# inhavl-shlee/AFI-GAN

Hardware: AMD Instinct MI355X
Metric: stage1_G+D_step_images_per_s (higher is better)
Workload: dtype f32 via f16x3: two scaled fp16 pieces per operand, three f16 MFMAs per product, fp32 accumulate (tensors fp32)

## Files before the change

afigan_amd/_lib.py:

```python
import ctypes as C
import os

import torch

_HERE = os.path.dirname(os.path.abspath(__file__))
LIB_PATH = os.environ.get("AFI_LIB_PATH") or os.path.join(_HERE, "csrc", "libafigan_hip.so")

AFI_MAX_RDB = 8
ABI_VERSION = 8


class AfiError(RuntimeError):
    pass


class View(C.Structure):
    _fields_ = [("p", C.c_void_p), ("sN", C.c_longlong), ("sH", C.c_longlong), ("sW", C.c_longlong)]


class GenParams(C.Structure):
    _fields_ = [("C", C.c_int), ("G", C.c_int), ("n_rdb", C.c_int), ("residual_scale", C.c_float),
                ("w0", C.c_void_p), ("b0", C.c_void_p),
                ("rdb_w", (C.c_void_p * 5) * AFI_MAX_RDB),
                ("w7", C.c_void_p), ("b7", C.c_void_p),
# ... 59 lines not shown
    "afi_conv1x1_wgrad": (_i, [_vp, View, View, _i, _i, _i, _i, _i, _vp, _f, _vp]),
    "afi_conv3x3_wino_ws_floats": (_ll, [_i] * 5),
    "afi_conv3x3_wino_fwd": (_i, [_vp, View, _i, _i, _i, _i, _vp, _vp, _i, View, _vp, _ll, _vp]),
    "afi_conv3x3_wino_infer": (_i, [_vp, View, _i, _i, _i, _i, _vp, _vp, _i, View, _i, _vp, _ll, _vp]),
    "afi_conv3x3_wino_dgrad": (_i, [_vp, View, _i, _i, _i, _i, _vp, _i, View, View, _vp, _ll, _vp]),
    "afi_conv3x3_wino_wgrad": (_i, [_vp, View, View, _i, _i, _i, _i, _i, _vp, _f, _vp, _ll, _vp]),
    "afi_conv3x3s2_fwd": (_i, [_vp, View, _i, _i, _i, _i, _vp, _vp, _i, View, _i, View, _f, View, _f, _vp]),
    "afi_conv3x3s2_dgrad": (_i, [_vp, View, _i, _i, _i, _i, _vp, _i, View, _f, _f, _vp]),
    "afi_conv3x3s2_wgrad": (_i, [_vp, View, View, _i, _i, _i, _i, _i, _vp, _f, _vp]),
    "afi_relu_bwd": (_i, [_vp, _vp, _vp, _ll, _f, _vp]),
    "afi_dwconv3x3_fwd": (_i, [View, _i, _i, _i, _i, _vp, _vp, _vp]),
    "afi_maxpool3s2_same_fwd": (_i, [View, _i, _i, _i, _i, _vp, _vp]),
    "afi_fuse_swish_fwd": (_i, [_vp, _vp, _vp, _vp, _vp, _ll, _vp]),
    "afi_fuse_swish_bwd_scratch_floats": (_ll, []),
    "afi_fuse_swish_bwd": (_i, [_vp, _vp, _vp, _vp, _vp, _vp, _vp, _vp, _vp, _ll, _vp, _vp]),
    "afi_dwconv3x3_wgrad_scratch_floats": (_ll, [_i]),
    "afi_dwconv3x3_wgrad": (_i, [_vp, _vp, _i, _i, _i, _i, _vp, _vp, _vp]),
    "afi_maxpool3s2_same_fwd_idx": (_i, [View, _i, _i, _i, _i, _vp, _vp, _vp]),
    "afi_maxpool3s2_same_bwd": (_i, [_vp, _vp, _i, _i, _i, _i, _vp, _vp]),
    "afi_bn_stats_ex": (_i, [_vp, _ll, _i, _f, _f, _vp, _vp, _vp, _vp, _vp, _vp, _vp, _vp]),
    "afi_bn_apply_fwd": (_i, [_vp, _vp, _vp, _vp, _vp, _vp, _ll, _i, _f, _vp]),
    "afi_resize_bilinear_u8_ws_bytes": (_ll, [_i, _i, _i, _i, _i]),
    "afi_resize_bilinear_u8": (_i, [_vp, _i, _i, _i, _vp, _i, _i, _i, _i, _vp, _ll, _vp]),
    "afi_dual_scale_u8_ws_bytes": (_ll, [_i, _i, _i, _i, _i, _i, _i]),
    "afi_dual_scale_u8": (_i, [_vp, _i, _i, _i, _vp, _i, _i, _i, _vp, _i, _i, _i, _i, _vp, _ll, _vp]),
    "afi_normalize_pad_u8": (_i, [_vp, _i, _i, _i, _vp, _vp, _vp, _i, _i, _vp]),
    "afi_convT6s2_pack_weight": (_i, [_vp, _vp, _i, _i, _vp]),
    "afi_convT6s2_unpack_wgrad": (_i, [_vp, _vp, _i, _i, _vp]),
    "afi_convT6s2_fwd": (_i, [_vp, View, _i, _i, _i, _i, _vp, _vp, _i, View, _i, _vp]),
    "afi_convT6s2_dgrad": (_i, [_vp, View, _i, _i, _i, _i, _vp, _i, View, View, _vp]),
    "afi_convT6s2_wgrad": (_i, [_vp, View, View, _i, _i, _i, _i, _i, _vp, _f, _vp]),
    "afi_bilinear2x_add_fwd": (_i, [View, _i, _i, _i, _i, _f, _vp, _vp]),
    "afi_bilinear2x_add_bwd": (_i, [_vp, _i, _i, _i, _i, _f, _vp, _vp]),
    "afi_reduce_scratch_floats": (_ll, [_i]),
    "afi_bn_stats": (_i, [_vp, _ll, _i, _vp, _vp, _vp, _vp, _vp, _vp, _vp]),
    "afi_bn_apply_lrelu_fwd": (_i, [_vp, _vp, _vp, _vp, _vp, _vp, _ll, _i, _vp]),
    "afi_bn_bwd": (_i, [_vp, _vp, _vp, _vp, _vp, _vp, _vp, _vp, _ll, _i, _vp, _vp]),
    "afi_bn_bwd_sums": (_i, [_vp, _vp, _vp, _vp, _vp, _vp, _vp, _ll, _i, _vp, _vp]),
    "afi_bn_bwd_apply": (_i, [_vp, _vp, _vp, _vp, _vp, _vp, _vp, _ll, _ll, _i, _vp]),
    "afi_colsum_accum": (_i, [_vp, _ll, _i, _ll, _f, _vp, _vp, _vp]),
    "afi_bce_logits_fwd_bwd": (_i, [_vp, _ll, _f, _f, _vp, _f, _vp, _vp]),
    "afi_l1_fwd_bwd": (_i, [View, View, _i, _i, _i, _i, _i, _i, _f, _vp, _f, _vp, _vp]),
    "afi_sgd_momentum_step": (_i, [_vp, _i, _ll, _f, _f, _f, _vp]),
    "afi_scale_inplace": (_i, [_vp, _ll, _f, _vp]),
    "afi_nchw_to_nhwc": (_i, [_vp, _vp, _i, _i, _i, _vp]),
    "afi_nhwc_to_nchw": (_i, [_vp, _vp, _i, _i, _i, _vp]),
    "afi_profile_enable": (_i, [_i]),
    "afi_profile_num_kinds": (_i, []),
    "afi_profile_kind_name": (C.c_char_p, [_i]),
    "afi_profile_get": (_i, [_i, C.POINTER(C.c_double)]),
    "afi_profile_dump": (_i, [C.c_char_p]),
    "afi_debug_wk6_convT_images": (_i, [_vp, _i, _i, _i, _vp, _vp, _vp, _vp, C.POINTER(C.c_longlong), _vp]),
    "afi_debug_wgrad_sk_plan": (_i, [C.POINTER(C.c_longlong), C.POINTER(C.c_int), _i, _i, C.POINTER(C.c_int), C.POINTER(C.c_int), C.POINTER(C.c_int)]),
}

_lib = None


def load():
    global _lib
    if _lib is not None:
        return _lib
    if not os.path.exists(LIB_PATH):
        raise AfiError(f"{LIB_PATH} not found: build it with `python __graft_entry__.py` (hipcc --offload-arch=gfx950). "
                       "There is no CPU fallback for the AFI-GAN hot path.")
    lib = C.CDLL(LIB_PATH)
    for name, (res, args) in SIGNATURES.items():
        fn = getattr(lib, name)
        fn.restype = res
        fn.argtypes = args
    if lib.afi_abi_version() != ABI_VERSION:
        raise AfiError(f"ABI mismatch: library {lib.afi_abi_version()} != binding {ABI_VERSION}")
    if not os.environ.get("AFI_LIB_PATH"):
        want, have = tree_digest(), lib.afi_build_id().decode()
        if want is not None and have != want:
            raise AfiError(f"{LIB_PATH} was built from other sources than this tree (library {have[:16]}, tree {want[:16]}): "
                           "rebuild it with `python -c 'import __graft_entry__ as g; g.build()'`")
    _lib = lib
    return lib


def tree_digest():
    import glob
    import hashlib
    csrc = os.path.join(_HERE, "csrc")
    hdr = os.path.join(os.path.dirname(_HERE), "include", "afigan_hip.h")
    files = sorted(glob.glob(os.path.join(csrc, "*.hip")) + [f for f in glob.glob(os.path.join(csrc, "*.h")) if os.path.basename(f) != "afi_build_id.h"])
    if not files or not os.path.exists(hdr):
        return None
    h = hashlib.sha256()
    for f in files + [hdr]:
        h.update(os.path.basename(f).encode() + b"\0")
        h.update(open(f, "rb").read())
    return h.hexdigest()


def build_id():
    return load().afi_build_id().decode()


def check(status: int, what: str = ""):
    if status != 0:
        msg = load().afi_status_string(status).decode()
        raise AfiError(f"{what or 'afigan_hip call'} failed: status {status} ({msg})")


# ... 134 lines not shown
```

afigan_amd/csrc/afi_gemm_f16.h:

```cpp
#pragma once

#include "afi_f16_split.h"
__device__ __forceinline__ f16x8 afi_tr_frag_f16(const unsigned char* base, int off_lo, int off_hi) {
    return __builtin_bit_cast(f16x8, afi_tr_frag(base, off_lo, off_hi));
}

__device__ __forceinline__ float afi_wave_max(float m) {
#pragma unroll
    for (int o = 32; o > 0; o >>= 1) m = fmaxf(m, __shfl_xor(m, o));
    return m;
}
__device__ __forceinline__ void afi_block_amax_publish(float m, float* slot) {
    __shared__ float red[16];
    m = afi_wave_max(m);
    const int lane = threadIdx.x & 63, wave = threadIdx.x >> 6, nw = (blockDim.x + 63) >> 6;
    if (lane == 0) red[wave] = m;
    __syncthreads();
    if (threadIdx.x == 0) {
        for (int w = 1; w < nw; ++w) m = fmaxf(m, red[w]);
        const unsigned bits = __float_as_uint(m);
        const unsigned cur = __hip_atomic_load((const unsigned*)slot, __ATOMIC_RELAXED, __HIP_MEMORY_SCOPE_AGENT);
        if (bits > cur) (void)atomicMax((unsigned*)slot, bits);
    }
}
// ... 531 lines not shown
        for (int ni = 0; ni < NI; ++ni) {
            bh[ni] = afi_tr_frag_f16(cur, fb_off[ni][0], fb_off[ni][1]);
            bl[ni] = afi_tr_frag_f16(cur + PART, fb_off[ni][0], fb_off[ni][1]);
        }
#pragma unroll
        for (int ni = 0; ni < NI; ++ni)
#pragma unroll
            for (int mi = 0; mi < MI; ++mi) acc[mi][ni] = mm(al[mi], bh[ni], acc[mi][ni]);
#pragma unroll
        for (int ni = 0; ni < NI; ++ni)
#pragma unroll
            for (int mi = 0; mi < MI; ++mi) acc[mi][ni] = mm(ah[mi], bl[ni], acc[mi][ni]);
#pragma unroll
        for (int ni = 0; ni < NI; ++ni)
#pragma unroll
            for (int mi = 0; mi < MI; ++mi) acc[mi][ni] = mm(ah[mi], bh[ni], acc[mi][ni]);
        asm volatile("s_waitcnt lgkmcnt(0)" ::: "memory");
    }
    const bool use_atomic = gridDim.y > 1;
    float* out = p.dU + (long long)plane * p.M * p.N;
    const long long ldn = p.N;
    if (use_atomic) {
#pragma unroll
        for (int mi = 0; mi < MI; ++mi)
#pragma unroll
            for (int ni = 0; ni < NI; ++ni)
#pragma unroll
                for (int r = 0; r < 16; ++r) {
                    const int row = m0 + (wm * MI + mi) * 32 + (r & 3) + 8 * (r >> 2) + 4 * lh;
                    __builtin_amdgcn_global_atomic_fadd_f32((__attribute__((address_space(1))) float*)(out + (long long)row * ldn + n0 + (wn * NI + ni) * 32 + lr),
                                                            (acc[mi][ni][r] * inv_q) * inv_v);
                }
    } else {
#pragma unroll
        for (int mi = 0; mi < MI; ++mi) {
            float old[NI][16];
#pragma unroll
            for (int ni = 0; ni < NI; ++ni)
#pragma unroll
                for (int r = 0; r < 16; ++r) {
                    const int row = m0 + (wm * MI + mi) * 32 + (r & 3) + 8 * (r >> 2) + 4 * lh;
                    old[ni][r] = out[(long long)row * ldn + n0 + (wn * NI + ni) * 32 + lr];
                }
#pragma unroll
            for (int ni = 0; ni < NI; ++ni)
#pragma unroll
                for (int r = 0; r < 16; ++r) {
                    const int row = m0 + (wm * MI + mi) * 32 + (r & 3) + 8 * (r >> 2) + 4 * lh;
                    out[(long long)row * ldn + n0 + (wn * NI + ni) * 32 + lr] = old[ni][r] + (acc[mi][ni][r] * inv_q) * inv_v;
                }
        }
    }
}
```

afigan_amd/csrc/igemm.hip:

```cpp
#include "afi_common.h"

#define AFI_BK 32
#define AFI_LDK (AFI_BK + 4)


__device__ __attribute__((aligned(16))) float afi_zeros[4] = {0.f, 0.f, 0.f, 0.f};

#include "afi_epilogue.h"

template <bool POST>
__global__ __launch_bounds__(256) void afi_pix_splitk_epilogue_kernel(const AfiPixGemm p) {
    const int HW = p.H * p.W;
    const long long M = (long long)p.N * HW;
    const int ldp = (p.Ncols + 3) & ~3;
    const int C_F4 = ldp >> 2;
    const long long total = M * C_F4;
    for (long long it = (long long)blockIdx.x * 256 + threadIdx.x; it < total; it += (long long)gridDim.x * 256) {
        const long long m = it / C_F4;
        const int col = (int)(it - m * C_F4) * 4;
        f32x4 v = {0.f, 0.f, 0.f, 0.f};
        const float* src = p.partial + m * ldp + col;
        const long long slab = M * ldp;
        int ks = 0;
        for (; ks + 4 <= p.splitK; ks += 4) {
// ... 478 lines not shown
    const long long ldn = p.N;
    if (use_atomic) {
#pragma unroll
        for (int mi = 0; mi < MI; ++mi)
#pragma unroll
            for (int r = 0; r < 16; ++r) {
                const int row = m0 + MI * ((r & 3) + 8 * (r >> 2) + 4 * lh) + mi;
                atomicAdd(out + (long long)row * ldn + n0 + wn * 32 + lr, acc[mi][r]);
            }
    } else {
        float old[MI][16];
#pragma unroll
        for (int mi = 0; mi < MI; ++mi)
#pragma unroll
            for (int r = 0; r < 16; ++r) {
                const int row = m0 + MI * ((r & 3) + 8 * (r >> 2) + 4 * lh) + mi;
                old[mi][r] = out[(long long)row * ldn + n0 + wn * 32 + lr];
            }
#pragma unroll
        for (int mi = 0; mi < MI; ++mi)
#pragma unroll
            for (int r = 0; r < 16; ++r) {
                const int row = m0 + MI * ((r & 3) + 8 * (r >> 2) + 4 * lh) + mi;
                out[(long long)row * ldn + n0 + wn * 32 + lr] = old[mi][r] + acc[mi][r];
            }
    }
}

#include <vector>
#include <atomic>
#include <mutex>
namespace {
struct ProfRec { hipEvent_t a, b; int kind; double flops; long long m; int n, k, split, planes; };
struct ProfState {
    std::atomic<bool> on{false};
    std::mutex mu;
    std::vector<ProfRec> recs;
    std::vector<hipEvent_t> pool;
    size_t used = 0;
} g_prof;
const char* kKindNames[] = {
    "pix_gemm<128x128,KC,linear> (1x1 / ragged-map / non-aligned Winograd GEMMs)", "pix_gemm<128x64,KC>", "pix_gemm<128x32,KC>", "pix_gemm<64x64,KC>",
    "pix_gemm<128x128,RC,linear> (conv dgrad, mid-size / ragged maps)", "pix_gemm<128x64,RC>", "pix_gemm<128x32,RC>", "pix_gemm<64x64,RC>",
    "wgrad_gemm<128x128>", "wgrad_gemm<64x128>", "wgrad_gemm<32x128>",
    "pix_gemm<128x128,KC,halo> (conv fwd)", "pix_gemm<128x128,RC,halo> (conv dgrad)",
    "gemm_nt<128x128> (batched Winograd GEMM)", "gemm_tn<128x128> (Winograd weight-gradient GEMM)",
    "pix_gemm_wk (small-map pixel GEMM, K split inside the block; grouped launches included)",
    "wgrad_group (grouped weight gradients of a small-map backward pass)",
    "gemm_nt_bf16<128x128> (batched Winograd GEMM on the bf16 MFMA: bf16x6 / bf16x3 / bf16 operands, fp32 accumulate)",
    "gemm_tn_bf16<128x128> (Winograd weight-gradient GEMM on the bf16 MFMA: bf16x6 / bf16x3 / bf16 operands, fp32 accumulate)",
    "wgrad_group6 (grouped weight gradients of a small-map backward pass on the bf16 MFMA, bf16x6 operands, fp32 accumulate)",
    "pix_gemm_wk6 (small-map pixel GEMM on the bf16 MFMA, bf16x6 operands on pre-split weight images, fp32 accumulate; grouped launches included)",
    "gemm_nt_f16x3 (batched Winograd GEMM on the f16 MFMA, 256x256 tiles where the grid fills the chip and 128x128 below: two scaled fp16 pieces per operand, three products, fp32 accumulate)",
    "gemm_tn_f16x3<128x128> (Winograd weight-gradient GEMM on the f16 MFMA: two scaled fp16 pieces per operand, three products, fp32 accumulate)"};
constexpr int kNumKinds = 23;
hipEvent_t prof_event() {
    if (g_prof.used == g_prof.pool.size()) {
        hipEvent_t e;
        (void)hipEventCreate(&e);
        g_prof.pool.push_back(e);
    }
    return g_prof.pool[g_prof.used++];
}
struct ProfScope {
    hipStream_t st; int kind; double flops; hipEvent_t a{};
    long long m = 0; int n = 0, k = 0, split = 1, planes = 1;
    ProfScope(hipStream_t s, int kd, double f) : st(s), kind(kd), flops(f) {
        if (g_prof.on) { std::lock_guard<std::mutex> lk(g_prof.mu); a = prof_event(); (void)hipEventRecord(a, st); started = true; }
    }
    bool live = true, started = false;
    void cancel() { live = false; }
    ~ProfScope() {
        if (started && live) { std::lock_guard<std::mutex> lk(g_prof.mu); hipEvent_t b = prof_event(); (void)hipEventRecord(b, st); g_prof.recs.push_back({a, b, kind, flops, m, n, k, split, planes}); }
    }
};
}

extern "C" int afi_profile_enable(int on) {
    std::lock_guard<std::mutex> lk(g_prof.mu);
    if (on) { g_prof.recs.clear(); g_prof.used = 0; }
    g_prof.on = on != 0;
    return AFI_OK;
}
extern "C" int afi_profile_num_kinds(void) { return kNumKinds; }
extern "C" const char* afi_profile_kind_name(int kind) { return (kind >= 0 && kind < kNumKinds) ? kKindNames[kind] : ""; }
extern "C" int afi_profile_get(int kind, double* out) {
    out[0] = out[1] = out[2] = 0.0;
    for (const ProfRec& r : g_prof.recs) {
        if (r.kind != kind) continue;
        if (hipEventSynchronize(r.b) != hipSuccess) return AFI_ERR_LAUNCH;
        float ms = 0.f;
        if (hipEventElapsedTime(&ms, r.a, r.b) != hipSuccess) return AFI_ERR_LAUNCH;
        out[0] += 1.0; out[1] += ms; out[2] += r.flops;
    }
    return AFI_OK;
}

#include <stdio.h>
extern "C" int afi_profile_dump(const char* path) {
    FILE* f = fopen(path, "w");
    if (!f) return AFI_ERR_BAD_ARG;
    fprintf(f, "kind,rows,cols,k,split,planes,ms,tflops\n");
    for (const ProfRec& r : g_prof.recs) {
        float ms = 0.f;
        if (hipEventSynchronize(r.b) != hipSuccess || hipEventElapsedTime(&ms, r.a, r.b) != hipSuccess) { fclose(f); return AFI_ERR_LAUNCH; }
        fprintf(f, "\"%s\",%lld,%d,%d,%d,%d,%.4f,%.2f\n", kKindNames[r.kind], r.m, r.n, r.k, r.split, r.planes, ms, ms > 0.f ? r.flops / (ms * 1e-3) / 1e12 : 0.0);
    }
// ... 161 lines not shown
                             bool a_pre, long long nt256_min_tiles, bool local_sums) {
    if (planes <= 0 || planes > 36 || rows_per_plane <= 0 || N <= 0 || K <= 0 || !ab.amax) return AFI_ERR_BAD_ARG;
    if ((rows_per_plane % 128) || (N % 128) || (K % 32)) return AFI_ERR_UNSUPPORTED;
    AfiGemmNT g{A, (const float*)Bimg, C, rows_per_plane, planes, N, K};
    const long long M = rows_per_plane * planes;
    const int ntm = (int)(M / 128), ntn = N / 128, chunk = afi_cdiv(ntm, 8);
    const size_t stage = 16384u + 2u * 8192u, epi = sizeof(float) * 64u * (128u + 4u);
    const size_t lds = stage > epi ? stage : epi;
    ProfScope prof(st, 21, 2.0 * (double)M * N * K);
    prof.m = M; prof.n = N; prof.k = K; prof.split = 2; prof.planes = planes;
    const int tpp = afi_cdiv(rows_per_plane, 256);
    const long long tiles256 = (long long)planes * tpp * (N / 256);
    if (local_sums && a_pre && !(N % 256)) {
        if (!afi_opt_in_big_lds((const void*)afi_gemm_nt_f16x3_w16_kernel<true, true>)) return AFI_ERR_LAUNCH;
        const int ntm2 = planes * tpp, ntn2 = N / 256, chunk2 = afi_cdiv(ntm2, 8);
        prof.split = 7;
        hipLaunchKernelGGL((afi_gemm_nt_f16x3_w16_kernel<true, true>), dim3(chunk2 * ntn2 * 8), dim3(1024), 16 * 16 * 132 * 4, st, g, ab, ntn2, ntm2, chunk2, tpp);
        return hipGetLastError() == hipSuccess ? AFI_OK : AFI_ERR_LAUNCH;
    }
    if (nt256_min_tiles > 0 && !(g_nt_abl & 32) && !(N % 256) && tiles256 >= nt256_min_tiles) {
        if (!afi_opt_in_big_lds(a_pre ? (const void*)afi_gemm_nt_f16x3_w16_kernel<true> : (const void*)afi_gemm_nt_f16x3_w16_kernel<false>)) return AFI_ERR_LAUNCH;
        const int ntm2 = planes * tpp, ntn2 = N / 256, chunk2 = afi_cdiv(ntm2, 8);
        prof.split = a_pre ? 4 : 3;
        if (a_pre) hipLaunchKernelGGL(afi_gemm_nt_f16x3_w16_kernel<true>, dim3(chunk2 * ntn2 * 8), dim3(1024), 16 * 16 * 132 * 4, st, g, ab, ntn2, ntm2, chunk2, tpp);
        else hipLaunchKernelGGL(afi_gemm_nt_f16x3_w16_kernel<false>, dim3(chunk2 * ntn2 * 8), dim3(1024), 16 * 16 * 132 * 4, st, g, ab, ntn2, ntm2, chunk2, tpp);
        return hipGetLastError() == hipSuccess ? AFI_OK : AFI_ERR_LAUNCH;
    }
    if (a_pre) {
        prof.split = 5;
        hipLaunchKernelGGL((afi_gemm_nt_f16x3_kernel<4, 0, true>), dim3(chunk * ntn * 8), dim3(256), lds, st, g, ab, ntn, ntm, chunk);
        return hipGetLastError() == hipSuccess ? AFI_OK : AFI_ERR_LAUNCH;
    }
#ifdef AFI_ABLATIONS
    const int abl = g_nt_abl & 31;
    if (abl == 1) hipLaunchKernelGGL((afi_gemm_nt_f16x3_kernel<4, 1>), dim3(chunk * ntn * 8), dim3(256), lds, st, g, ab, ntn, ntm, chunk);
    else if (abl == 2) hipLaunchKernelGGL((afi_gemm_nt_f16x3_kernel<4, 2>), dim3(chunk * ntn * 8), dim3(256), lds, st, g, ab, ntn, ntm, chunk);
    else if (abl == 4) hipLaunchKernelGGL((afi_gemm_nt_f16x3_kernel<4, 4>), dim3(chunk * ntn * 8), dim3(256), lds, st, g, ab, ntn, ntm, chunk);
    else if (abl == 8) hipLaunchKernelGGL((afi_gemm_nt_f16x3_kernel<4, 8>), dim3(chunk * ntn * 8), dim3(256), lds, st, g, ab, ntn, ntm, chunk);
    else if (abl == 16) hipLaunchKernelGGL((afi_gemm_nt_f16x3_kernel<4, 16>), dim3(chunk * ntn * 8), dim3(256), lds, st, g, ab, ntn, ntm, chunk);
    else if (abl == 12) hipLaunchKernelGGL((afi_gemm_nt_f16x3_kernel<4, 12>), dim3(chunk * ntn * 8), dim3(256), lds, st, g, ab, ntn, ntm, chunk);
    else if (abl == 6) hipLaunchKernelGGL((afi_gemm_nt_f16x3_kernel<4, 6>), dim3(chunk * ntn * 8), dim3(256), lds, st, g, ab, ntn, ntm, chunk);
    else if (abl == 14) hipLaunchKernelGGL((afi_gemm_nt_f16x3_kernel<4, 14>), dim3(chunk * ntn * 8), dim3(256), lds, st, g, ab, ntn, ntm, chunk);
    else if (abl == 10) hipLaunchKernelGGL((afi_gemm_nt_f16x3_kernel<4, 10>), dim3(chunk * ntn * 8), dim3(256), lds, st, g, ab, ntn, ntm, chunk);
    else if (abl == 20) hipLaunchKernelGGL((afi_gemm_nt_f16x3_kernel<4, 20>), dim3(chunk * ntn * 8), dim3(256), lds, st, g, ab, ntn, ntm, chunk);
    else if (abl == 24) hipLaunchKernelGGL((afi_gemm_nt_f16x3_kernel<4, 24>), dim3(chunk * ntn * 8), dim3(256), lds, st, g, ab, ntn, ntm, chunk);
    else
#endif
    hipLaunchKernelGGL((afi_gemm_nt_f16x3_kernel<4>), dim3(chunk * ntn * 8), dim3(256), lds, st, g, ab, ntn, ntm, chunk);
    return hipGetLastError() == hipSuccess ? AFI_OK : AFI_ERR_LAUNCH;
}
#ifndef AFI_TN_MAX_ROUNDS
#define AFI_TN_MAX_ROUNDS 6
#endif
int afi_launch_gemm_tn_f16x3(const float* Q, const float* V, float* dU, int planes, long long rows_per_plane, int M, int N, const AfiF16Bound& qb, const AfiF16Bound& vb,
                             hipStream_t st, bool pre, bool deterministic) {
    if (planes <= 0 || planes > 36 || rows_per_plane <= 0 || M <= 0 || N <= 0 || !qb.amax || !vb.amax) return AFI_ERR_BAD_ARG;
    if ((rows_per_plane % 32) || (M % 128) || (N % 128)) return AFI_ERR_UNSUPPORTED;
    const int ntm = M / 128, ntn = N / 128;
    const long long tiles = (long long)ntm * ntn * planes;
    const int slots = AFI_TN_WAVES == 8 ? 768 : (AFI_TN_RING == 3 ? 768 : (AFI_TN_RING == 2 ? 1024 : 512));
    int splitK = 1;
    {
        const int maxsplit = (int)(rows_per_plane / (16 * 32)) > 0 ? (int)(rows_per_plane / (16 * 32)) : 1;
        double best = -1.0;
        for (int s2 = 1; s2 <= maxsplit && s2 <= 128; ++s2) {
            const long long blocks = tiles * s2;
            if (blocks < 2 * slots && s2 < maxsplit) continue;
            if (blocks > AFI_TN_MAX_ROUNDS * slots && best >= 0.0) break;
            const long long rounds = (blocks + slots - 1) / slots;
            const double fill = (double)blocks / (double)(rounds * slots);
            if (fill > best + 1e-3) { best = fill; splitK = s2; }
        }
    }
    if (deterministic) splitK = 1;
    int kper = (int)((rows_per_plane + splitK - 1) / splitK);
    kper = ((kper + 31) / 32) * 32;
    splitK = (int)((rows_per_plane + kper - 1) / kper);
    AfiGemmTN g{Q, V, dU, rows_per_plane, planes, M, N};
    ProfScope prof(st, 22, 2.0 * (double)rows_per_plane * planes * M * N);
    prof.m = (long long)M * planes; prof.n = N; prof.k = (int)rows_per_plane; prof.split = splitK; prof.planes = planes;
    if (pre) hipLaunchKernelGGL(afi_gemm_tn_f16x3_pre_kernel, dim3((unsigned)tiles, splitK), dim3(64 * AFI_TN_WAVES), (unsigned)AFI_TN_RING * 4u * 4096u, st, g, qb, vb, ntm, ntn, kper);
    else hipLaunchKernelGGL(afi_gemm_tn_f16x3_kernel, dim3((unsigned)tiles, splitK), dim3(256), 2u * 4u * 4096u, st, g, qb, vb, ntm, ntn, kper);
    return hipGetLastError() == hipSuccess ? AFI_OK : AFI_ERR_LAUNCH;
}
int afi_launch_pix_gemm_sk(const AfiPixGemm& p, int b_rc, hipStream_t st);
int afi_launch_pix_gemm_wk_group(const AfiPixGemm* probs, int n, int b_rc, hipStream_t st);
int afi_launch_wgrad_group(const AfiWgradGemm* probs, int n, int wide, hipStream_t st);
int afi_launch_wgrad6_group(const AfiWgradGemm* probs, int n, hipStream_t st);
int afi_launch_pix_gemm_group(const AfiPixGemm* probs, int n, int b_rc, hipStream_t st) {
    double fl = 0.0; long long m = 0; int nn = 0;
    for (int i = 0; i < n; ++i) {
        const long long M = (long long)probs[i].N * probs[i].H * probs[i].W;
        fl += 2.0 * (double)M * probs[i].Ncols * probs[i].ntaps * probs[i].nKphase * probs[i].Ck;
        m = M; nn += probs[i].Ncols;
    }
    bool all6 = n > 0;
    for (int i = 0; i < n; ++i) all6 = all6 && probs[i].Bimg != nullptr;
    ProfScope prof(st, all6 ? 20 : 15, fl);
    prof.m = m; prof.n = nn; prof.k = n > 0 ? probs[0].ntaps * probs[0].nKphase * probs[0].Ck : 0;
    const int rc = afi_launch_pix_gemm_wk_group(probs, n, b_rc, st);
    if (rc == AFI_ERR_UNSUPPORTED) prof.cancel();
    return rc;
}
int afi_launch_wgrad_gemm_group(const AfiWgradGemm* probs, int n, int wide, hipStream_t st) {
    if (n <= 0) return AFI_OK;
    double fl = 0.0;
    for (int i = 0; i < n; ++i) fl += 2.0 * (double)probs[i].N * probs[i].H * probs[i].W * probs[i].Mrows * probs[i].Ncols * probs[i].ntaps;
    ProfScope prof(st, 16, fl);
    prof.m = n;
    return afi_launch_wgrad_group(probs, n, wide, st);
}
int afi_launch_wgrad_gemm_group6(const AfiWgradGemm* probs, int n, hipStream_t st) {
    if (n <= 0) return AFI_OK;
    double fl = 0.0;
    for (int i = 0; i < n; ++i) fl += 2.0 * (double)probs[i].N * probs[i].H * probs[i].W * probs[i].Mrows * probs[i].Ncols * probs[i].ntaps;
    ProfScope prof(st, 19, fl);
    prof.m = n; prof.split = 6;
    const int rc = afi_launch_wgrad6_group(probs, n, st);
    if (rc == AFI_ERR_UNSUPPORTED) prof.cancel();
    return rc;
}
int afi_launch_pix_gemm(const AfiPixGemm& p_in, int b_rc, hipStream_t st) {
    AfiPixGemm p = p_in;
    const long long M = (long long)p.N * p.H * p.W;
    if (M <= 0 || p.Ncols <= 0 || p.Ck <= 0) return AFI_ERR_BAD_ARG;
    if (p.a_bn.mean) return AFI_ERR_UNSUPPORTED;
    if (p.b_sImg != 0 && ((long long)p.H * p.W) % 128 != 0) return AFI_ERR_BAD_ARG;
    if (b_rc && (p.Ncols & 3)) return AFI_ERR_UNSUPPORTED;
    if (!b_rc && (p.Ck & 3)) return AFI_ERR_UNSUPPORTED;
    if (p.gtap) {
        if (p.ntaps < 1 || p.ntaps > 9 || p.a_sgn != 1 || p.nKphase != 1 || (p.a_stride != 1 && p.a_stride != 2)) return AFI_ERR_BAD_ARG;
        const bool small = M <= 64 * 256 || p.Ncols <= 64;
        if (!b_rc) return small ? launch_pix<64, 64, 2, 2, false, AFI_BK, false, true>(p, st) : launch_pix<128, 128, 2, 2, false, AFI_BK, false, true>(p, st);
        return small ? launch_pix<64, 64, 2, 2, true, AFI_BK, false, true>(p, st) : launch_pix<128, 128, 2, 2, true, AFI_BK, false, true>(p, st);
    }
    if (p.ntaps != 1 && p.ntaps != 9) return AFI_ERR_BAD_ARG;
// ... 140 lines not shown
```

afigan_amd/csrc/nets.hip:

```cpp
#include <string.h>
#include <stdlib.h>

#include "../../include/afigan_hip.h"
#include "afi_common.h"
#include <initializer_list>
#include <new>

int afi_launch_pix_gemm(const AfiPixGemm& p, int b_rc, hipStream_t st);
int afi_launch_gemm_tn(const float* Q, const float* V, float* dU, int planes, long long rows_per_plane, int M, int N, hipStream_t st, bool deterministic = false);
int afi_launch_gemm_nt(const float* A, const float* B, float* C, int planes, long long rows_per_plane, int N, int K, hipStream_t st);
int afi_launch_split_bf16_tiles(const float* B, void* out, int planes, int N, int K, int split, hipStream_t st);
int afi_launch_gemm_nt_bf16_dma(const float* A, const void* Bsplit, float* C, int planes, long long rows_per_plane, int N, int K, int split, hipStream_t st);
int afi_launch_gemm_tn_bf16(const float* Q, const float* V, float* dU, int planes, long long rows_per_plane, int M, int N, int split, hipStream_t st, bool deterministic = false);
int afi_launch_split_f16_tiles(const float* B, void* out, int planes, int N, int K, hipStream_t st, int wkind = 0);
int afi_f16_image_begin(void* out, hipStream_t st);
float* afi_f16_image_wmax(void* out);
long long afi_f16_image_bytes(int planes, int N, int K);
int afi_launch_absmax_planes(const float* X, long long per_plane, int planes, float* out, hipStream_t st);
AfiF16Bound afi_f16_bound(const float* amax, int kind);
int afi_launch_gemm_nt_f16x3(const float* A, const void* Bimg, float* C, int planes, long long rows_per_plane, int N, int K, const AfiF16Bound& ab, hipStream_t st,
                             bool a_pre = false, long long nt256_min_tiles = 512, bool local_sums = false);
int afi_launch_gemm_tn_f16x3(const float* Q, const float* V, float* dU, int planes, long long rows_per_plane, int M, int N, const AfiF16Bound& qb, const AfiF16Bound& vb,
                             hipStream_t st, bool pre = false, bool deterministic = false);
int afi_launch_wgrad_gemm(const AfiWgradGemm& p, hipStream_t st);
int afi_launch_wgrad_gemm_group(const AfiWgradGemm* probs, int n, int wide, hipStream_t st);
int afi_launch_wgrad_gemm_group6(const AfiWgradGemm* probs, int n, hipStream_t st);
int afi_launch_colsum_group(const AfiColsumProb* probs, int n, hipStream_t st);
int afi_launch_pix_gemm_group(const AfiPixGemm* probs, int n, int b_rc, hipStream_t st);
long long afi_wk6_image_bytes(int Ncols, int Ck, int ntaps, int nKphase);
int afi_launch_wk6_images(const AfiWk6ImgJob* jobs, int n, hipStream_t st, const AfiWk6Side* side, const AfiWk6ConvT* ct);
int afi_launch_rdb_chain6(const AfiChain6& c, hipStream_t st);
int afi_launch_nchw_to_nhwc(const float* in, float* out, int N, int C, int P, hipStream_t st);
int afi_launch_nhwc_to_nchw(const float* in, float* out, int N, int C, int P, hipStream_t st);
int afi_launch_convT_pack(const float* W, float* Wp, int Cin, int Cout, hipStream_t st);
int afi_launch_convT_unpack_grad(const float* dWp, float* dW, int Cin, int Cout, hipStream_t st);
int afi_launch_rdb_wgrad_unpack(const float* dWp, float* const dw[4], int C, int G, float alpha, hipStream_t st);
int afi_launch_rdb_wgrad_unpack_multi(const float* dWp, long long stride, float* const (*dw)[4], int nblocks, int C, int G, float alpha, hipStream_t st);
int afi_launch_g_bwd_tail(const AfiColsumProb* cs, int n_cs, const float* dWpT, float* dWT, int Cin, int Cout,
                          const float* dWp, long long stride, float* const (*dw)[4], int nblocks, int C, int G, float alpha, hipStream_t st);
int afi_launch_rdb_xpart_pack(const float* const w[4], float* out, int C, int G, hipStream_t st);
int afi_launch_lrelu_slice(AfiView v, int N, int H, int W, int nch, hipStream_t st);
int afi_launch_bn_stats(const float* x, long long P, int C, float* mean, float* invstd, float* var_out, float* running_mean,
                        float* running_var, float* scratch, hipStream_t st, long long* num_batches_tracked = nullptr, float eps = -1.f,
                        float momentum = -1.f, bool fp64 = true);
int afi_launch_bn_stats_from_partials(const double* partial, int rows, long long P, int C, float* mean, float* invstd, float* var_out, float* running_mean,
                                      float* running_var, hipStream_t st, long long* num_batches_tracked = nullptr, float eps = -1.f, float momentum = -1.f);
int afi_launch_view_absmax(AfiView x, int N, int H, int W, int C, float* amax, hipStream_t st);
int afi_launch_bn_act_amax(const float* mm, int rows, int C, const float* mean, const float* invstd, const float* gamma, const float* beta, float slope,
                           float* amax, hipStream_t st);
int afi_wino_stats_rows(long long T, int C);
#ifndef AFI_STATS_MAX_ROWS
#define AFI_STATS_MAX_ROWS 1024
#endif
int afi_launch_bn_apply_lrelu(const float* x, float* y, const float* mean, const float* invstd, const float* gamma, const float* beta,
                              long long P, int C, hipStream_t st, float slope = AFI_LRELU_SLOPE, float* amax = nullptr);
int afi_launch_bn_bwd(const float* g, const float* x, float* dx, const float* mean, const float* invstd, const float* gamma, float* dgamma,
                      float* dbeta, float gscale, long long P, int C, float* scratch, hipStream_t st, const float* mask_beta = nullptr,
                      float slope = AFI_LRELU_SLOPE, float* amax = nullptr);
int afi_launch_colsum_accum(const float* g, long long P, int C, long long ld, float alpha, float* db, float* scratch, hipStream_t st);
int afi_launch_bn_bwd_sums(const float* g, const float* x, const float* mean, const float* invstd, float* dgamma, float* dbeta, float* sums2C, long long P, int C,
                           float* scratch, hipStream_t st);
int afi_launch_bn_bwd_apply(const float* g, const float* x, float* dx, const float* mean, const float* invstd, const float* gamma, const float* sums2C, long long P,
                            long long P_total, int C, hipStream_t st);
int afi_launch_stencil9_sum(const float* d9, int ld, const float* bias, float* out, int N, int H, int W, hipStream_t st);
int afi_launch_stencil9_scatter(const float* dlogit, float* dd9, int ld, int N, int H, int W, hipStream_t st);
int afi_launch_bn_bwd_from_partials(const double* partial, int rows, const float* g, const float* x, float* dx, const float* mean, const float* invstd,
                                    const float* gamma, float* dgamma, float* dbeta, float gscale, long long P, int C, float* scratch, hipStream_t st,
                                    const float* mask_beta, float slope, float* amax);
extern "C" long long afi_disc_tail_scratch_floats(int C);
int afi_launch_disc_tail_fwd(const float* x, const AfiBnLoad* bn, float slope, const float* w3, float* d9, long long P, int C, hipStream_t st);
int afi_launch_disc_tail_bwd(const float* x, const float* dd9, const AfiBnLoad bn, float slope, const float* w3, float* dx, float* dgamma, float* dbeta, float* dw3,
                             long long P, int C, float* scratch, float* amax, hipStream_t st);
int afi_launch_bce_logits(const float* z, long long n, float target, float lscale, float* loss, float gscale, float* dz, hipStream_t st);
int afi_launch_l1(AfiView a, AfiView b, int N, int h, int w, int C, int Ha, int Wa, float lscale, float* loss, float gscale, float* da,
                  hipStream_t st);
int afi_launch_bilinear2x_fwd(AfiView x, int N, int H, int W, int C, float beta, float* out, hipStream_t st);
// ... 1826 lines not shown
```

include/afigan_hip.h:

```cpp
#ifndef AFIGAN_HIP_H
#define AFIGAN_HIP_H

#include <stddef.h>
#include <stdint.h>

#ifdef __cplusplus
extern "C" {
#endif

#define AFI_OK 0
#define AFI_ERR_BAD_ARG 1
#define AFI_ERR_UNSUPPORTED 2
#define AFI_ERR_LAUNCH 3
#define AFI_ERR_WORKSPACE 4

#define AFI_MAX_RDB 8

typedef struct afi_view {
    float* p;
    long long sN, sH, sW;
} afi_view_t;

int afi_abi_version(void);
const char* afi_status_string(int status);
// ... 143 lines not shown
int afi_convT6s2_dgrad(afi_ctx_t* ctx, afi_view_t dy , int N, int H, int W, int Cout, const float* wp, int Cin,
                       afi_view_t dx, afi_view_t z_or_null, void* stream);
int afi_convT6s2_wgrad(afi_ctx_t* ctx, afi_view_t dy, afi_view_t x, int N, int H, int W, int Cout, int Cin, float* dwp, float alpha, void* stream);

int afi_bilinear2x_add_fwd(afi_view_t x, int N, int H, int W, int C, float beta, float* out, void* stream);
int afi_bilinear2x_add_bwd(const float* dout, int N, int H, int W, int C, float beta, float* dx, void* stream);

long long afi_reduce_scratch_floats(int C);
int afi_bn_stats(const float* x, long long P, int C, float* mean, float* invstd, float* var_biased_or_null,
                 float* running_mean_or_null, float* running_var_or_null, float* scratch, void* stream);
int afi_bn_apply_lrelu_fwd(const float* x, float* y, const float* mean, const float* invstd, const float* gamma,
                           const float* beta, long long P, int C, void* stream);
int afi_bn_stats_ex(const float* x, long long P, int C, float eps, float momentum, float* mean, float* invstd, float* var_biased_or_null,
                    float* running_mean_or_null, float* running_var_or_null, long long* num_batches_tracked_or_null, float* scratch,
                    void* stream);
int afi_bn_apply_fwd(const float* x, float* y, const float* mean, const float* invstd, const float* gamma, const float* beta,
                     long long P, int C, float slope, void* stream);
int afi_bn_bwd(const float* g, const float* x, float* dx, const float* mean, const float* invstd, const float* gamma,
               float* dgamma, float* dbeta, long long P, int C, float* scratch, void* stream);
int afi_bn_bwd_sums(const float* g, const float* x, const float* mean, const float* invstd, float* dgamma_or_null, float* dbeta_or_null, float* sums2C,
                    long long P, int C, float* scratch, void* stream);
int afi_bn_bwd_apply(const float* g, const float* x, float* dx, const float* mean, const float* invstd, const float* gamma, const float* sums2C,
                     long long P, long long P_total, int C, void* stream);
int afi_colsum_accum(const float* g, long long P, int C, long long ld, float alpha, float* db, float* scratch, void* stream);

int afi_bce_logits_fwd_bwd(const float* z, long long n, float target, float lscale, float* loss, float gscale, float* dz, void* stream);
int afi_l1_fwd_bwd(afi_view_t a, afi_view_t b, int N, int h, int w, int C, int Ha, int Wa, float lscale, float* loss,
                   float gscale, float* da, void* stream);

typedef struct afi_sgd_desc { float* p; const float* g; float* m; long long n; float wd; float pad_; } afi_sgd_desc_t;
int afi_sgd_momentum_step(const afi_sgd_desc_t* descs_dev, int ntensors, long long max_n, float lr, float momentum,
                          float gscale, void* stream);
int afi_scale_inplace(float* p, long long n, float s, void* stream);

int afi_nchw_to_nhwc(const float* in, float* out, int N, int C, int P, void* stream);
int afi_nhwc_to_nchw(const float* in, float* out, int N, int C, int P, void* stream);

long long afi_resize_bilinear_u8_ws_bytes(int H0, int W0, int C, int H1, int W1);
int afi_resize_bilinear_u8(const unsigned char* src, int H0, int W0, int C, unsigned char* dst, int H1, int W1, int hflip,
                           int out_chw, void* ws, long long ws_bytes, void* stream);
long long afi_dual_scale_u8_ws_bytes(int H0, int W0, int C, int H1, int W1, int H2, int W2);
int afi_dual_scale_u8(const unsigned char* src, int H0, int W0, int C, unsigned char* image, int H1, int W1, int hflip,
                      unsigned char* image_r, int H2, int W2, int hflip_r, int out_chw, void* ws, long long ws_bytes, void* stream);
int afi_normalize_pad_u8(const unsigned char* img_chw, int C, int H, int W, const float* mean, const float* std_,
                         float* out, int Hp, int Wp, void* stream);

int afi_profile_enable(int on);
int afi_profile_num_kinds(void);
const char* afi_profile_kind_name(int kind);
int afi_profile_get(int kind, double* out3);
int afi_profile_dump(const char* path);

int afi_debug_wgrad_sk_plan(const long long* pixels, const int* tiles, int nprob, int bpc, int* stored, int* added, int* stages);
int afi_debug_wk6_convT_images(const float* W, int Cin, int Cout, int mode, void* direct, float* pack_ride, void* via_pack, float* pack_ref,
                               long long* bytes, void* stream);

#ifdef __cplusplus
}
#endif
#endif
```

Baseline: 28.72.

## Add 256x128 tall-tile f16x3 weight-gradient GEMM kernel for pre-split planes

Adds an 8-wave, 256x128 tile variant of the Winograd weight-gradient f16x3 GEMM with a three-stage LDS ring fed by direct global-to-LDS loads. The planner picks it when the operands are pre-split and M is a multiple of 256, which halves how often each V tile is reloaded per output row block. It also recomputes split-K against a smaller slot count. Costs are more LDS per block, lower occupancy, and fewer blocks for the grid to spread across the chip. Debug entry points for the plan and the kernel are added.

```diff
diff --git a/afigan_amd/_lib.py b/afigan_amd/_lib.py
--- a/afigan_amd/_lib.py
+++ b/afigan_amd/_lib.py
@@ -135,6 +135,8 @@
     "afi_profile_dump": (_i, [C.c_char_p]),
     "afi_debug_wk6_convT_images": (_i, [_vp, _i, _i, _i, _vp, _vp, _vp, _vp, C.POINTER(C.c_longlong), _vp]),
     "afi_debug_wgrad_sk_plan": (_i, [C.POINTER(C.c_longlong), C.POINTER(C.c_int), _i, _i, C.POINTER(C.c_int), C.POINTER(C.c_int), C.POINTER(C.c_int)]),
+    "afi_debug_tn_f16x3_plan": (_i, [_i, _ll, _i, _i, _i, _i, C.POINTER(C.c_int)]),
+    "afi_debug_gemm_tn_f16x3_pre": (_i, [_vp, _vp, _vp, _i, _ll, _i, _i, _vp, _vp, _i, _i, _vp]),
 }
 
 _lib = None
diff --git a/afigan_amd/csrc/afi_gemm_f16.h b/afigan_amd/csrc/afi_gemm_f16.h
--- a/afigan_amd/csrc/afi_gemm_f16.h
+++ b/afigan_amd/csrc/afi_gemm_f16.h
@@ -607,3 +607,143 @@
         }
     }
 }
+
+__global__ __launch_bounds__(512, 4) void afi_gemm_tn_f16x3_tall_kernel(const AfiGemmTN p, const AfiF16Bound qb, const AfiF16Bound vb, int ntile_m, int ntile_n, int kper) {
+    constexpr int BM = 256, BN = 128, HK = 16, WN = 2, MI = 2, NI = 2, RING = 3;
+    constexpr int PART = HK * 128 * 2;
+    constexpr int BUF = 6 * PART;
+    extern __shared__ __attribute__((aligned(16))) unsigned char smem_b[];
+    const int tid = threadIdx.x, lane = tid & 63, wave = __builtin_amdgcn_readfirstlane(tid >> 6);
+    const int wm = wave / WN, wn = wave % WN;
+    const int lr = lane & 31, lh = lane >> 5;
+    int t;
+    {
+        const int nwg = gridDim.x, q = nwg >> 3, r = nwg & 7, xcd = blockIdx.x & 7;
+        t = (xcd < r ? xcd * (q + 1) : r * (q + 1) + (xcd - r) * q) + (blockIdx.x >> 3);
+    }
+    const int tile_n = t % ntile_n; t /= ntile_n;
+    const int tile_m = t % ntile_m; const int plane = t / ntile_m;
+    const int m0 = tile_m * BM, n0 = tile_n * BN;
+    const long long k_begin = (long long)blockIdx.y * kper;
+    const long long k_end = (k_begin + kper < p.rows_per_plane) ? k_begin + kper : p.rows_per_plane;
+    if (k_begin >= k_end) return;
+    const int nH = (int)((k_end - k_begin) / HK);
+    typedef __attribute__((address_space(3))) void* lptr;
+    const unsigned char* src[3];
+    int voff[3], dst_off[3];
+    long long step[3];
+#pragma unroll
+    for (int j = 0; j < 3; ++j) {
+        const int g = 3 * wave + j, I = g >> 2, i = g & 3;
+        const int op = I >> 2, piece = op ? I & 1 : (I >> 1) & 1, col0 = op ? n0 : m0 + 128 * (I & 1);
+        const long long ld = op ? p.N : p.M;
+        src[j] = (const unsigned char*)((op ? p.V : p.Q) + ((long long)plane * p.rows_per_plane + k_begin + 4 * i) * ld) + (long long)(col0 >> 5) * 128 + piece * 64;
+        const int ch = (lane & 15) ^ (((lane >> 4) << 2) | i);
+        voff[j] = (lane >> 4) * (int)(ld * 4) + (ch >> 2) * 128 + (ch & 3) * 16;
+        dst_off[j] = I * PART + i * 1024;
+        step[j] = (long long)HK * ld * 4;
+    }
+    const unsigned lds_base = (unsigned)(unsigned long long)(lptr)smem_b;
+    auto issue = [&](int h) {
+        const unsigned dst = lds_base + (unsigned)((h % RING) * BUF);
+#pragma unroll
+        for (int j = 0; j < 3; ++j) {
+            const unsigned char* gsrc = src[j] + (long long)h * step[j] + voff[j];
+            unsigned keep;
+            asm volatile("s_mov_b32 %0, m0\n\ts_mov_b32 m0, %2\n\ts_nop 0\n\tglobal_load_lds_dwordx4 %1, off\n\ts_mov_b32 m0, %0"
+                         : "=&s"(keep) : "v"(gsrc), "s"(dst + (unsigned)dst_off[j]) : "memory");
+        }
+    };
+    issue(0);
+    if (1 < nH) issue(1);
+    const float s_q = afi_f16_scale(qb.amax[(long long)plane * qb.stride] * qb.cmul[plane]);
+    const float s_v = afi_f16_scale(vb.amax[(long long)plane * vb.stride] * vb.cmul[plane]);
+    const float inv_q = afi_pow2_inverse(s_q), inv_v = afi_pow2_inverse(s_v);
+    int fa_off[MI][2], fb_off[NI][2];
+    {
+        const int g = lane >> 4, i = lane & 15, q = i >> 2, pp = i & 3;
+#pragma unroll
+        for (int rd = 0; rd < 2; ++rd) {
+            const int r = 8 * (g >> 1) + 4 * rd + q;
+            const int swz = ((r & 3) << 2) | ((r >> 2) & 3);
+#pragma unroll
+            for (int mi = 0; mi < MI; ++mi) fa_off[mi][rd] = (wm >> 1) * PART + 256 * r + 16 * ((4 * ((wm & 1) * MI + mi) + 2 * (g & 1) + (pp >> 1)) ^ swz) + 8 * (pp & 1);
+#pragma unroll
+            for (int ni = 0; ni < NI; ++ni) fb_off[ni][rd] = 4 * PART + 256 * r + 16 * ((4 * (wn * NI + ni) + 2 * (g & 1) + (pp >> 1)) ^ swz) + 8 * (pp & 1);
+        }
+    }
+    f32x16 acc[MI][NI];
+#pragma unroll
+    for (int mi = 0; mi < MI; ++mi)
+#pragma unroll
+        for (int ni = 0; ni < NI; ++ni)
+#pragma unroll
+            for (int r = 0; r < 16; ++r) acc[mi][ni][r] = 0.f;
+    auto mm = [](f16x8 x, f16x8 y, f32x16 c) -> f32x16 { return __builtin_amdgcn_mfma_f32_32x32x16_f16(x, y, c, 0, 0, 0); };
+
+    for (int h = 0; h < nH; ++h) {
+        if (h + 1 < nH) asm volatile("s_waitcnt vmcnt(3)" ::: "memory");
+        else asm volatile("s_waitcnt vmcnt(0)" ::: "memory");
+        __builtin_amdgcn_s_barrier();
+        if (h + 2 < nH) issue(h + 2);
+        const unsigned char* cur = smem_b + (h % RING) * BUF;
+        f16x8 ah[MI], al[MI], bh[NI], bl[NI];
+#pragma unroll
+        for (int mi = 0; mi < MI; ++mi) {
+            ah[mi] = afi_tr_frag_f16(cur, fa_off[mi][0], fa_off[mi][1]);
+            al[mi] = afi_tr_frag_f16(cur + 2 * PART, fa_off[mi][0], fa_off[mi][1]);
+        }
+#pragma unroll
+        for (int ni = 0; ni < NI; ++ni) {
+            bh[ni] = afi_tr_frag_f16(cur, fb_off[ni][0], fb_off[ni][1]);
+            bl[ni] = afi_tr_frag_f16(cur + PART, fb_off[ni][0], fb_off[ni][1]);
+        }
+#pragma unroll
+        for (int ni = 0; ni < NI; ++ni)
+#pragma unroll
+            for (int mi = 0; mi < MI; ++mi) acc[mi][ni] = mm(al[mi], bh[ni], acc[mi][ni]);
+#pragma unroll
+        for (int ni = 0; ni < NI; ++ni)
+#pragma unroll
+            for (int mi = 0; mi < MI; ++mi) acc[mi][ni] = mm(ah[mi], bl[ni], acc[mi][ni]);
+#pragma unroll
+        for (int ni = 0; ni < NI; ++ni)
+#pragma unroll
+            for (int mi = 0; mi < MI; ++mi) acc[mi][ni] = mm(ah[mi], bh[ni], acc[mi][ni]);
+        asm volatile("s_waitcnt lgkmcnt(0)" ::: "memory");
+    }
+    const bool use_atomic = gridDim.y > 1;
+    float* out = p.dU + (long long)plane * p.M * p.N;
+    const long long ldn = p.N;
+    if (use_atomic) {
+#pragma unroll
+        for (int mi = 0; mi < MI; ++mi)
+#pragma unroll
+            for (int ni = 0; ni < NI; ++ni)
+#pragma unroll
+                for (int r = 0; r < 16; ++r) {
+                    const int row = m0 + (wm * MI + mi) * 32 + (r & 3) + 8 * (r >> 2) + 4 * lh;
+                    __builtin_amdgcn_global_atomic_fadd_f32((__attribute__((address_space(1))) float*)(out + (long long)row * ldn + n0 + (wn * NI + ni) * 32 + lr),
+                                                            (acc[mi][ni][r] * inv_q) * inv_v);
+                }
+    } else {
+#pragma unroll
+        for (int mi = 0; mi < MI; ++mi) {
+            float old[NI][16];
+#pragma unroll
+            for (int ni = 0; ni < NI; ++ni)
+#pragma unroll
+                for (int r = 0; r < 16; ++r) {
+                    const int row = m0 + (wm * MI + mi) * 32 + (r & 3) + 8 * (r >> 2) + 4 * lh;
+                    old[ni][r] = out[(long long)row * ldn + n0 + (wn * NI + ni) * 32 + lr];
+                }
+#pragma unroll
+            for (int ni = 0; ni < NI; ++ni)
+#pragma unroll
+                for (int r = 0; r < 16; ++r) {
+                    const int row = m0 + (wm * MI + mi) * 32 + (r & 3) + 8 * (r >> 2) + 4 * lh;
+                    out[(long long)row * ldn + n0 + (wn * NI + ni) * 32 + lr] = old[ni][r] + (acc[mi][ni][r] * inv_q) * inv_v;
+                }
+        }
+    }
+}
diff --git a/afigan_amd/csrc/igemm.hip b/afigan_amd/csrc/igemm.hip
--- a/afigan_amd/csrc/igemm.hip
+++ b/afigan_amd/csrc/igemm.hip
@@ -554,7 +554,7 @@
     "wgrad_group6 (grouped weight gradients of a small-map backward pass on the bf16 MFMA, bf16x6 operands, fp32 accumulate)",
     "pix_gemm_wk6 (small-map pixel GEMM on the bf16 MFMA, bf16x6 operands on pre-split weight images, fp32 accumulate; grouped launches included)",
     "gemm_nt_f16x3 (batched Winograd GEMM on the f16 MFMA, 256x256 tiles where the grid fills the chip and 128x128 below: two scaled fp16 pieces per operand, three products, fp32 accumulate)",
-    "gemm_tn_f16x3<128x128> (Winograd weight-gradient GEMM on the f16 MFMA: two scaled fp16 pieces per operand, three products, fp32 accumulate)"};
+    "gemm_tn_f16x3 (Winograd weight-gradient GEMM on the f16 MFMA, 256x128 tiles on pre-split planes where M allows and 128x128 otherwise: two scaled fp16 pieces per operand, three products, fp32 accumulate)"};
 constexpr int kNumKinds = 23;
 hipEvent_t prof_event() {
     if (g_prof.used == g_prof.pool.size()) {
@@ -822,19 +822,22 @@
 #ifndef AFI_TN_MAX_ROUNDS
 #define AFI_TN_MAX_ROUNDS 6
 #endif
-int afi_launch_gemm_tn_f16x3(const float* Q, const float* V, float* dU, int planes, long long rows_per_plane, int M, int N, const AfiF16Bound& qb, const AfiF16Bound& vb,
-                             hipStream_t st, bool pre, bool deterministic) {
-    if (planes <= 0 || planes > 36 || rows_per_plane <= 0 || M <= 0 || N <= 0 || !qb.amax || !vb.amax) return AFI_ERR_BAD_ARG;
-    if ((rows_per_plane % 32) || (M % 128) || (N % 128)) return AFI_ERR_UNSUPPORTED;
-    const int ntm = M / 128, ntn = N / 128;
-    const long long tiles = (long long)ntm * ntn * planes;
-    const int slots = AFI_TN_WAVES == 8 ? 768 : (AFI_TN_RING == 3 ? 768 : (AFI_TN_RING == 2 ? 1024 : 512));
+#ifndef AFI_TN_TALL
+#define AFI_TN_TALL 1
+#endif
+struct AfiTnPlan { int tall, bm, splitK, kper; long long tiles; };
+static AfiTnPlan afi_tn_f16x3_plan(int planes, long long rows_per_plane, int M, int N, bool pre, bool deterministic, bool allow_tall = true) {
+    AfiTnPlan pl;
+    pl.tall = AFI_TN_TALL && allow_tall && pre && AFI_TN_WAVES == 4 && AFI_TN_RING == 2 && !(M % 256);
+    pl.bm = pl.tall ? 256 : 128;
+    pl.tiles = (long long)(M / pl.bm) * (N / 128) * planes;
+    const int slots = pl.tall ? 512 : AFI_TN_WAVES == 8 ? 768 : (AFI_TN_RING == 3 ? 768 : (AFI_TN_RING == 2 ? 1024 : 512));
     int splitK = 1;
     {
         const int maxsplit = (int)(rows_per_plane / (16 * 32)) > 0 ? (int)(rows_per_plane / (16 * 32)) : 1;
         double best = -1.0;
         for (int s2 = 1; s2 <= maxsplit && s2 <= 128; ++s2) {
-            const long long blocks = tiles * s2;
+            const long long blocks = pl.tiles * s2;
             if (blocks < 2 * slots && s2 < maxsplit) continue;
             if (blocks > AFI_TN_MAX_ROUNDS * slots && best >= 0.0) break;
             const long long rounds = (blocks + slots - 1) / slots;
@@ -845,13 +848,38 @@
     if (deterministic) splitK = 1;
     int kper = (int)((rows_per_plane + splitK - 1) / splitK);
     kper = ((kper + 31) / 32) * 32;
-    splitK = (int)((rows_per_plane + kper - 1) / kper);
+    pl.splitK = (int)((rows_per_plane + kper - 1) / kper);
+    pl.kper = kper;
+    return pl;
+}
+extern "C" int afi_debug_tn_f16x3_plan(int planes, long long rows_per_plane, int M, int N, int pre, int deterministic, int* out) {
+    if (!out || planes <= 0 || rows_per_plane <= 0 || (rows_per_plane % 32) || M <= 0 || N <= 0 || (M % 128) || (N % 128)) return AFI_ERR_BAD_ARG;
+    const AfiTnPlan pl = afi_tn_f16x3_plan(planes, rows_per_plane, M, N, pre != 0, deterministic != 0);
+    out[0] = pl.tall; out[1] = pl.bm; out[2] = pl.splitK; out[3] = pl.kper;
+    return AFI_OK;
+}
+int afi_launch_gemm_tn_f16x3(const float* Q, const float* V, float* dU, int planes, long long rows_per_plane, int M, int N, const AfiF16Bound& qb, const AfiF16Bound& vb,
+                             hipStream_t st, bool pre, bool deterministic, bool allow_tall) {
+    if (planes <= 0 || planes > 36 || rows_per_plane <= 0 || M <= 0 || N <= 0 || !qb.amax || !vb.amax) return AFI_ERR_BAD_ARG;
+    if ((rows_per_plane % 32) || (M % 128) || (N % 128)) return AFI_ERR_UNSUPPORTED;
+    const AfiTnPlan pl = afi_tn_f16x3_plan(planes, rows_per_plane, M, N, pre, deterministic, allow_tall);
+    const int ntm = M / pl.bm, ntn = N / 128, splitK = pl.splitK, kper = pl.kper;
+    const long long tiles = pl.tiles;
     AfiGemmTN g{Q, V, dU, rows_per_plane, planes, M, N};
     ProfScope prof(st, 22, 2.0 * (double)rows_per_plane * planes * M * N);
     prof.m = (long long)M * planes; prof.n = N; prof.k = (int)rows_per_plane; prof.split = splitK; prof.planes = planes;
-    if (pre) hipLaunchKernelGGL(afi_gemm_tn_f16x3_pre_kernel, dim3((unsigned)tiles, splitK), dim3(64 * AFI_TN_WAVES), (unsigned)AFI_TN_RING * 4u * 4096u, st, g, qb, vb, ntm, ntn, kper);
+    if (pl.tall) {
+        if (!afi_opt_in_big_lds((const void*)afi_gemm_tn_f16x3_tall_kernel)) return AFI_ERR_LAUNCH;
+        hipLaunchKernelGGL(afi_gemm_tn_f16x3_tall_kernel, dim3((unsigned)tiles, splitK), dim3(512), 3u * 6u * 4096u, st, g, qb, vb, ntm, ntn, kper);
+    } else if (pre) hipLaunchKernelGGL(afi_gemm_tn_f16x3_pre_kernel, dim3((unsigned)tiles, splitK), dim3(64 * AFI_TN_WAVES), (unsigned)AFI_TN_RING * 4u * 4096u, st, g, qb, vb, ntm, ntn, kper);
     else hipLaunchKernelGGL(afi_gemm_tn_f16x3_kernel, dim3((unsigned)tiles, splitK), dim3(256), 2u * 4u * 4096u, st, g, qb, vb, ntm, ntn, kper);
     return hipGetLastError() == hipSuccess ? AFI_OK : AFI_ERR_LAUNCH;
+}
+extern "C" int afi_debug_gemm_tn_f16x3_pre(const void* Q, const void* V, float* dU, int planes, long long rows_per_plane, int M, int N, const float* qmax,
+                                           const float* vmax, int deterministic, int kernel, void* stream) {
+    if (!Q || !V || !dU || !qmax || !vmax || kernel < 0 || kernel > 1) return AFI_ERR_BAD_ARG;
+    return afi_launch_gemm_tn_f16x3((const float*)Q, (const float*)V, dU, planes, rows_per_plane, M, N, afi_f16_bound(qmax, 0), afi_f16_bound(vmax, 0),
+                                    (hipStream_t)stream, true, deterministic != 0, kernel == 0);
 }
 int afi_launch_pix_gemm_sk(const AfiPixGemm& p, int b_rc, hipStream_t st);
 int afi_launch_pix_gemm_wk_group(const AfiPixGemm* probs, int n, int b_rc, hipStream_t st);
diff --git a/afigan_amd/csrc/nets.hip b/afigan_amd/csrc/nets.hip
--- a/afigan_amd/csrc/nets.hip
+++ b/afigan_amd/csrc/nets.hip
@@ -21,7 +21,7 @@
 int afi_launch_gemm_nt_f16x3(const float* A, const void* Bimg, float* C, int planes, long long rows_per_plane, int N, int K, const AfiF16Bound& ab, hipStream_t st,
                              bool a_pre = false, long long nt256_min_tiles = 512, bool local_sums = false);
 int afi_launch_gemm_tn_f16x3(const float* Q, const float* V, float* dU, int planes, long long rows_per_plane, int M, int N, const AfiF16Bound& qb, const AfiF16Bound& vb,
-                             hipStream_t st, bool pre = false, bool deterministic = false);
+                             hipStream_t st, bool pre = false, bool deterministic = false, bool allow_tall = true);
 int afi_launch_wgrad_gemm(const AfiWgradGemm& p, hipStream_t st);
 int afi_launch_wgrad_gemm_group(const AfiWgradGemm* probs, int n, int wide, hipStream_t st);
 int afi_launch_wgrad_gemm_group6(const AfiWgradGemm* probs, int n, hipStream_t st);
diff --git a/include/afigan_hip.h b/include/afigan_hip.h
--- a/include/afigan_hip.h
+++ b/include/afigan_hip.h
@@ -219,6 +219,9 @@
 int afi_profile_dump(const char* path);
 
 int afi_debug_wgrad_sk_plan(const long long* pixels, const int* tiles, int nprob, int bpc, int* stored, int* added, int* stages);
+int afi_debug_tn_f16x3_plan(int planes, long long rows_per_plane, int M, int N, int pre, int deterministic, int* out);
+int afi_debug_gemm_tn_f16x3_pre(const void* Q, const void* V, float* dU, int planes, long long rows_per_plane, int M, int N, const float* qmax,
+                                const float* vmax, int deterministic, int kernel, void* stream);
 int afi_debug_wk6_convT_images(const float* W, int Cin, int Cout, int mode, void* direct, float* pack_ride, void* via_pack, float* pack_ref,
                                long long* bytes, void* stream);
 
```

After: 29.05 (median of 6 runs). +1.2%, better.
